# rchiaramo/wavefront_path_tracer

Measured on AMD Instinct MI355X. Metric: Mrays/s (extend+shade) at 1920×1080, 64 spp, 8 bounces; 1/2/4/8 GPU, higher is better.
Workload: dtype f32

## Files before the change

### wavefront_path_tracer_amd/_build.py

```python
import os
import shutil
import subprocess

PKG_DIR = os.path.dirname(os.path.abspath(__file__))
ROOT = os.path.dirname(PKG_DIR)
CSRC = os.path.join(PKG_DIR, "csrc")
LIB_PATH = os.path.join(PKG_DIR, "libwfpt.so")
SOURCES = ["wfpt_kernels.hip", "wfpt_api.hip", "wfpt_bvh_build.hip", "wfpt_host.cpp"]
HEADERS = [os.path.join(CSRC, "wfpt_kernels.h"), os.path.join(CSRC, "wfpt_bvh4.h"), os.path.join(CSRC, "wfpt_device_math.h"), os.path.join(CSRC, "wfpt_tile_lists.h"), os.path.join(CSRC, "wfpt_first_schedule.h"),
           os.path.join(ROOT, "include", "wfpt.h")]
FLAGS = ["--offload-arch=gfx950", "-O3", "-std=c++17", "-fPIC", "-shared", "-ffp-contract=off",
         "-fhip-fp32-correctly-rounded-divide-sqrt", "-fno-fast-math", "-Wall", "-Wno-unused-function"]


def hipcc():
    exe = shutil.which("hipcc") or "/opt/rocm/bin/hipcc"
    if not os.path.exists(exe):
        raise RuntimeError("hipcc not found: libwfpt.so cannot be built (and there is no CPU fallback)")
    return exe


def stale():
    if not os.path.exists(LIB_PATH):
        return True
    t = os.path.getmtime(LIB_PATH)
    deps = [os.path.join(CSRC, s) for s in SOURCES] + HEADERS + [os.path.abspath(__file__)]
    return any(os.path.getmtime(d) > t for d in deps)


BUILD_INFO = os.path.join(PKG_DIR, "build_info.json")


def source_digest():
    import hashlib
    h = hashlib.sha256()
    for f in [os.path.join(CSRC, s) for s in SOURCES] + HEADERS:
        h.update(os.path.basename(f).encode() + b"\0")
        h.update(open(f, "rb").read())
    return h.hexdigest()


def write_build_info():
    import datetime
    import json

    def git(*a):
        try:
            return subprocess.run(["git", "-C", ROOT] + list(a), stdout=subprocess.PIPE, stderr=subprocess.DEVNULL, text=True, timeout=20).stdout.strip()
        except Exception:
            return ""
    info = {"git_head": git("rev-parse", "HEAD") or None, "git_dirty": bool(git("status", "--porcelain", "--untracked-files=no")),
            "built_utc": datetime.datetime.utcnow().strftime("%Y-%m-%dT%H:%M:%SZ"), "source_sha256": source_digest(),
            "flags": FLAGS + os.environ.get("WFPT_EXTRA_FLAGS", "").split()}
    try:
        json.dump(info, open(BUILD_INFO, "w"), indent=1)
    except OSError:
        pass
    return info


def build_info():
    import json
    try:
        info = json.load(open(BUILD_INFO))
    except Exception:
        info = {"git_head": None}
    try:
        info["sources_match_build"] = info.get("source_sha256") == source_digest()
    except OSError:
        info["sources_match_build"] = None
    return info


def build(force=False, verbose=False):
    if not force and not stale():
        return LIB_PATH
    out = os.environ.get("WFPT_LIB_OUT", LIB_PATH)
    cmd = [hipcc()] + FLAGS + os.environ.get("WFPT_EXTRA_FLAGS", "").split()
    cmd += ["-I" + os.path.join(ROOT, "include"), "-I" + CSRC, "-o", out]
    cmd += [os.path.join(CSRC, s) for s in SOURCES]
    if verbose:
        print(" ".join(cmd))
    res = subprocess.run(cmd, stdout=subprocess.PIPE, stderr=subprocess.STDOUT, text=True)
    if res.returncode != 0:
        raise RuntimeError("hipcc failed:\n" + res.stdout)
    if verbose and res.stdout.strip():
        print(res.stdout)
    if out == LIB_PATH:
        write_build_info()
    return out


if __name__ == "__main__":
    print(build(force=True, verbose=True))
```

### wavefront_path_tracer_amd/csrc/wfpt_kernels.h

```cpp
#pragma once
#include <hip/hip_runtime.h>
#include <stddef.h>
#include <stdint.h>

#include "wfpt.h"
#include "wfpt_bvh4.h"
#include "wfpt_device_math.h"
#include "wfpt_first_schedule.h"
#include "wfpt_tile_lists.h"

namespace wfpt {

#ifndef WFPT_CHUNK
#define WFPT_CHUNK 512
#endif
constexpr int kChunk = WFPT_CHUNK;
constexpr int kExtendThreads = kChunk;
constexpr int kExtendWaves = kExtendThreads / 64;
#ifndef WFPT_CONSUMER_THREADS
#define WFPT_CONSUMER_THREADS 256
#endif
constexpr int kConsumerThreads = WFPT_CONSUMER_THREADS;
constexpr int kScanThreads = 1024;
constexpr int kMaxRows = 64;
constexpr int kMaxTrailDepth = 63;
constexpr int kMaxBatch = 128;
constexpr int kClsMax = 8;
constexpr int kMaxBatchClassic = 64;

struct Stride32 {
    uint32_t v;
    __host__ __device__ operator size_t() const { return v; }
    __host__ __device__ Stride32 &operator=(size_t x) { v = static_cast<uint32_t>(x); return *this; }
};

struct RayQueue {
    float *base;
    uint32_t cap;
    __host__ __device__ float *ox() const { return base; }
    __host__ __device__ float *oy() const { return base + cap; }
    __host__ __device__ float *oz() const { return base + 2u * static_cast<size_t>(cap); }
    __host__ __device__ float *dx() const { return base + 3u * static_cast<size_t>(cap); }
    __host__ __device__ float *dy() const { return base + 4u * static_cast<size_t>(cap); }
    __host__ __device__ float *dz() const { return base + 5u * static_cast<size_t>(cap); }
    __host__ __device__ uint32_t *pixel() const { return reinterpret_cast<uint32_t *>(base + 6u * static_cast<size_t>(cap)); }
};

struct HitQueue {
    uint32_t *base;
    Stride32 plane;
    __host__ __device__ float *t() const { return reinterpret_cast<float *>(base); }
    __host__ __device__ uint32_t *prim() const { return base + static_cast<size_t>(plane); }
    __host__ __device__ uint32_t *ridx() const { return base + 2u * static_cast<size_t>(plane); }
};
struct MissQueue {
    uint32_t *base;
    Stride32 plane;
    __host__ __device__ uint32_t *ridx() const { return base; }
    __host__ __device__ float *dy() const { return reinterpret_cast<float *>(base + static_cast<size_t>(plane)); }
    __host__ __device__ uint32_t *pixel() const { return base + 2u * static_cast<size_t>(plane); }
    __host__ __device__ float *dx() const { return reinterpret_cast<float *>(base + 3u * static_cast<size_t>(plane)); }
    __host__ __device__ float *dz() const { return reinterpret_cast<float *>(base + 4u * static_cast<size_t>(plane)); }
};
constexpr uint32_t kMissPlanes = 3, kMissPlanesEnv = 5;

struct EnvDev {
    const float4 *texels;
    uint32_t w, h;
    float intensity, rotation;
};

constexpr uint32_t kNoTexture = 0xffffffffu;
struct TexScene {
    const uint2 *prim_tex;
    const TexDev *tex;
    const float *uv6;
};

struct Control {
    uint32_t counters[16];
    wfpt_frame_buffer frame;
    uint32_t n_in;
    uint32_t seg_n;
    uint32_t hits;
    uint32_t misses;
    uint32_t shade_n;
    uint32_t miss_n;
    uint32_t shade_gx;
    uint32_t done;
    uint32_t ticket;
    uint32_t bounce;
    uint32_t samples;
    uint32_t _pad;
    uint32_t cls_n[kClsMax];
    uint32_t n_segs, next_segs, _pad2[2];
    uint32_t rows[kMaxRows][4];
    unsigned long long totals[4];
    unsigned long long wave_totals[kMaxRows][3];
};

struct ShadeRec {
    float v[3];
    float fuzz;
    float albedo[3];
    float refract_index;
    uint32_t mat_type;
    uint32_t cost_class;
    uint32_t _pad[2];
};

struct SceneDev {
    const wfpt_bvh_node *nodes;
    const float4 *prim_geom;
    const uint16_t *pair_parent;
    const uint32_t *pair_parent32;
    const wfpt_sphere *spheres;
    const wfpt_triangle *triangles;
    const wfpt_material *materials;
    const float4 *shade_rec;
    uint32_t n_nodes, n_spheres, n_materials;
    uint32_t prim_kind;
    uint32_t lds_scene;
    uint32_t lds_bytes;
    uint32_t depth;
    const float4 *nodes4;
    uint32_t tile_n;
    uint32_t *stack_spill;
    uint32_t spill_stride;
    const float4 *nodes_ch;
    float safe_c[3], safe_r2;
    uint32_t exact;
    uint32_t root_leaf;
};

constexpr uint32_t kStack4Lds = 8;
constexpr uint32_t kTileNodesMax = 341;

struct CameraDev {
    wfpt_gpu_camera cam;
    float inv_proj[16];
    float view[16];
};

struct Tiling {
    uint32_t rank, world;
};

struct Batch {
    uint32_t n;
    uint32_t ctl_stride;
    Stride32 ray_stride;
    Stride32 queue_stride;
    Stride32 chunk_stride;
    Stride32 image_stride;
};

struct GenerateArgs {
    Batch batch;
    RayQueue q;
    float *image;
    Control *ctl;
    const CameraDev *camera;
    uint32_t gx, gy;
    uint32_t true_size;
    uint32_t reset_image;
    uint32_t set_n_in;
    uint32_t capacity;
    Tiling tile;
};

struct ExtendArgs {
    Batch batch;
    RayQueue q;
    HitQueue hq;
    MissQueue mq;
    uint32_t *chunk_hits, *chunk_miss;
    float4 *rec_out;
    Control *ctl;
    const uint32_t *n_in;
    uint32_t limit;
    uint32_t has_inactive;
    uint32_t partition;
    uint16_t *mat_list;
    uint32_t *chunk_mat;
    size_t mat_list_mstride;
    size_t chunk_mat_mstride;
    SceneDev scene;
};

struct ScanArgs {
    Batch batch;
    const uint32_t *chunk_hits, *chunk_miss;
    uint32_t *chunk_hit_base, *chunk_miss_base;
    Control *ctl;
    const uint32_t *n_in;
    uint32_t limit;
    uint32_t *first_seg;
    uint32_t fused;
    uint32_t miss_floor;
    uint32_t bounce;
};

constexpr int kBounceFirst = 0;
constexpr int kBounceMiddle = 1;
constexpr int kBounceLast = 2;
#ifndef WFPT_MISS_SEGS
#define WFPT_MISS_SEGS 16
#endif
constexpr int kMissSegsPerItem = WFPT_MISS_SEGS;
#ifndef WFPT_MISS_EVERY
#define WFPT_MISS_EVERY 0
#endif
constexpr uint32_t kMissEvery = WFPT_MISS_EVERY;
#ifndef WFPT_FIRST_STATIC_SHARE_NUM
#define WFPT_FIRST_STATIC_SHARE_NUM 1
#endif
#ifndef WFPT_FIRST_STATIC_SHARE_DEN
#define WFPT_FIRST_STATIC_SHARE_DEN 2
#endif
constexpr uint32_t kFirstStaticNum = WFPT_FIRST_STATIC_SHARE_NUM, kFirstStaticDen = WFPT_FIRST_STATIC_SHARE_DEN;
static_assert(kFirstStaticDen > 0 && kFirstStaticNum <= kFirstStaticDen, "the static share of the first launch's items lies in [0, 1]");

struct BounceArgs {
    Batch batch;
    unsigned long long *stamps;
    const float4 *rec_in;
    float4 *rec_out;
    const uint32_t *in_hits, *in_hit_base, *in_miss;
    const uint32_t *in_first_seg;
    uint32_t *out_hits, *out_miss;
    MissQueue mq_in, mq_out;
    float *image;
    Control *ctl;
    const CameraDev *camera;
    uint32_t gx, gy;
    uint32_t capacity;
    uint32_t rng_mode;
    uint32_t image_width;
    Tiling tile;
    SceneDev scene;
    const uint32_t *plan;
    uint32_t plan_seg_off, plan_miss_off;
    const uint2 *cls_table;
    const uint32_t *first_seg_cls;
    uint32_t *out_cls;
    const uint4 *tile_lists;
};

struct TileListArgs {
    const float4 *nodes_ch;
    uint32_t n_nodes;
    const CameraDev *camera;
    uint32_t gx, gy;
    uint32_t width, height;
    Tiling tile;
    uint32_t *records;
};

template <int K> struct ClsPack {
    static constexpr int kFields = K + 2, kWords = (kFields + 2) / 3;
};
constexpr int kBinClasses = 4;
static_assert(kBinClasses <= kClsMax && kChunk <= 1023, "a packed field must hold a segment's count");

struct ScanBinnedArgs {
    Batch batch;
    const uint32_t *chunk_hits, *chunk_miss, *chunk_cls;
    uint2 *cls_table;
    uint32_t *first_seg_cls;
    Control *ctl;
    const uint32_t *n_in;
    uint32_t limit, miss_floor, bounce;
};

struct PlanArgs {
    Batch batch;
    const Control *ctl;
    uint32_t *plan;
    uint32_t plan_seg_off, plan_miss_off;
    uint32_t last;
};

constexpr uint32_t kDenseMiss = 0xffffffffu, kDenseInactive = 0xfffffffeu;
#ifndef WFPT_TICKET_BLOCK
#define WFPT_TICKET_BLOCK 64
#endif
constexpr uint32_t kTicketBlock = WFPT_TICKET_BLOCK;
#ifndef WFPT_REFILL_IDLE_PRESHADED
#define WFPT_REFILL_IDLE_PRESHADED 24
#endif
#ifndef WFPT_REFILL_IDLE_FIRST_PRE
#define WFPT_REFILL_IDLE_FIRST_PRE 16
#endif
constexpr uint32_t kRefillIdlePreshaded = WFPT_REFILL_IDLE_PRESHADED, kRefillIdleFirstPre = WFPT_REFILL_IDLE_FIRST_PRE;

struct RefillArgs {
    Batch batch;
    unsigned long long *stamps;
    const float4 *rec_in;
    float4 *dense_out;
    const uint32_t *in_hits, *in_hit_base, *in_first_seg;
    float *image;
    Control *ctl;
    const CameraDev *camera;
    uint32_t gx, gy, capacity, rng_mode, image_width;
    Tiling tile;
    SceneDev scene;
};

struct CompactArgs {
    Batch batch;
    const float4 *dense_in;
    float4 *rec_out;
    MissQueue mq_out;
    uint32_t *out_hits, *out_miss;
    const Control *ctl;
    uint32_t capacity;
};

struct ShadeArgs {
    Batch batch;
    RayQueue q, ext;
    HitQueue hq;
    const uint32_t *chunk_hits, *chunk_hit_base;
    const float4 *rec_in;
    float *image;
    Control *ctl;
    const uint32_t *n_hits;
    uint32_t limit;
    uint32_t gx;
    uint32_t rng_mode;
    uint32_t material;
    uint32_t split;
    const uint16_t *mat_list;
    const uint32_t *chunk_mat;
    size_t mat_list_mstride, chunk_mat_mstride;
    uint32_t count_out;
    uint32_t image_width;
    SceneDev scene;
    Tiling tile;
};

struct MissArgs {
    Batch batch;
    RayQueue q;
    MissQueue mq;
    const uint32_t *chunk_miss, *chunk_miss_base;
    float *image;
    const Control *ctl;
    const uint32_t *n_miss;
    uint32_t limit;
    uint32_t image_width;
    Tiling tile;
};

struct HitWalk {
    Batch batch;
    const float4 *rec_in;
    const uint32_t *in_hits, *in_hit_base;
    RayQueue q;
    HitQueue hq;
    const uint32_t *n_hits;
    uint32_t limit;
    uint32_t material;
    uint32_t capacity;
    float *image;
    const Control *ctl;
    uint32_t image_width;
    Tiling tile;
    const float4 *shade_rec;
};

struct TextureArgs {
    HitWalk w;
// ... 196 lines not shown
```

### wavefront_path_tracer_amd/csrc/wfpt_kernels.hip

```cpp
#include "wfpt_kernels.h"
#include "wfpt_device_math.h"

#include <type_traits>

namespace wfpt {

namespace {

constexpr float kPi = 3.1415927f;

__device__ __forceinline__ uint32_t lane_id() { return threadIdx.x & 63u; }
__device__ __forceinline__ uint32_t mbcnt(unsigned long long mask) {
    return __builtin_amdgcn_mbcnt_hi(static_cast<uint32_t>(mask >> 32),
                                     __builtin_amdgcn_mbcnt_lo(static_cast<uint32_t>(mask), 0u));
}
__device__ __forceinline__ uint32_t umin(uint32_t a, uint32_t b) { return a < b ? a : b; }
__device__ __forceinline__ uint32_t umax(uint32_t a, uint32_t b) { return a > b ? a : b; }
__device__ __forceinline__ uint32_t uniform(uint32_t v) { return __builtin_amdgcn_readfirstlane(v); }

#define WFPT_AS_LDS __attribute__((address_space(3)))
#define WFPT_AS_GLOBAL __attribute__((address_space(1)))
typedef float v4f_ __attribute__((ext_vector_type(4)));
__device__ __forceinline__ float4 load4_lds(const float4 *p) {
    const v4f_ v = *(const WFPT_AS_LDS v4f_ *)p;
// ... 1748 lines not shown
    if (shade_stamps) { asm volatile("s_waitcnt vmcnt(0)" ::: "memory"); shade_stamps[1] = stamp_now(); }
#endif
    shade_record<SCATTER, true, true>(s, ra, rb, __float_as_uint(rb.w), h, fb, ox, oy, oz, dx, dy, dz, pixel_idx);
}

typedef uint32_t v4u_ __attribute__((ext_vector_type(4)));
#define WFPT_AS_CONSTANT __attribute__((address_space(4)))
template <int PRIM>
__device__ __forceinline__ bool trace_tile_list(const uint4 *record, uint32_t w0, const float4 *prim_geom, float ox, float oy, float oz, float dx,
                                                float dy, float dz, float &t_out, uint32_t &prim_out) {
    const float a = (dx * dx + dy * dy) + dz * dz;
    float nearest = 1e30f;
    uint32_t best = 0xffffffffu, best_leaf = 0;
    const WFPT_AS_CONSTANT v4u_ *rec = (const WFPT_AS_CONSTANT v4u_ *)reinterpret_cast<uintptr_t>(record);
    uint32_t w = w0;
    for (uint32_t q = 0; q < kTileListCap / 4u && w != 0u; ++q) {
        const v4u_ four = rec[q];
        const uint32_t ws[4] = {four.x, four.y, four.z, four.w};
#pragma unroll
        for (int k = 0; k < 4; ++k) {
            w = ws[k];
            if (w == 0u) break;
            visit_leaf<PRIM>(prim_geom, w & 0xffffu, w >> 16, w, ox, oy, oz, dx, dy, dz, a, nearest, best, best_leaf);
        }
    }
    leaf_box_verdict<PRIM>(prim_geom, best_leaf & 0xffffu, best_leaf >> 16, false, ox, oy, oz, dx, dy, dz, nearest, best);
    t_out = nearest;
    prim_out = best;
    return nearest < 1e30f;
}

constexpr int kTileListThreads = 256;
__global__ __launch_bounds__(kTileListThreads) void tile_lists_kernel(TileListArgs a) {
    const uint32_t lane = lane_id();
    const uint32_t tile = uniform(blockIdx.x * (kTileListThreads / 64u) + (threadIdx.x >> 6));
    if (tile >= a.gx * a.gy) return;
    uint32_t *rec = a.records + static_cast<size_t>(tile) * kTileListCap;
    uint32_t x0, y0;
    tile_origin(tile, a.gx, a.tile.rank, a.tile.world, x0, y0);
    const CameraDev &cam = *a.camera;
    const TileBundle b = tile_bundle(cam.cam, cam.inv_proj, cam.view, x0, y0, a.width, a.height);
    bool list = b.ok != 0u && __float_as_uint(a.nodes_ch[1].w) == 0u;
    uint32_t count = 0;
    for (uint32_t base = 0; base < a.n_nodes && list; base += 64u) {
        const uint32_t i = base + lane;
        uint32_t w = 0u;
        if (i < a.n_nodes) {
            const float4 c = a.nodes_ch[2u * i], h = a.nodes_ch[2u * i + 1u];
            w = tile_leaf_word(i, __float_as_uint(c.w), __float_as_uint(h.w));
            if (w != 0u && w != kTileNoList && !tile_bundle_reaches(b, c.x, c.y, c.z, h.x, h.y, h.z)) w = 0u;
        }
        const unsigned long long mask = __ballot(w != 0u);
        const uint32_t slot = count + mbcnt(mask);
        if (__ballot(w == kTileNoList) != 0ull) list = false;
        if (w != 0u && slot < kTileListCap) rec[slot] = w;
        count += static_cast<uint32_t>(__popcll(mask));
        if (count > kTileListCap) list = false;
    }
    if (lane < kTileListCap) {
        if (!list) rec[lane] = lane == 0u ? kTileNoList : 0u;
        else if (lane >= count) rec[lane] = 0u;
    }
}

struct TicketMap {
    uint32_t n_hit, every, n_mixed;
    __device__ __forceinline__ TicketMap(uint32_t n_hit_items, uint32_t n_items, bool mix) : n_hit(n_hit_items) {
        const uint32_t n_miss = n_items - n_hit_items;
        every = kMissEvery ? kMissEvery : uniform(umin(umax(n_hit_items / umax(n_miss, 1u), 1u), 62u)) + 1u;
        n_mixed = mix ? umin(n_miss, n_hit_items / (every - 1u)) : 0u;
    }
    __device__ __forceinline__ uint32_t item_of(uint32_t t) const {
        if (t < n_mixed * every) {
            const uint32_t k = t / every, r = t - k * every;
            return r == every - 1u ? n_hit + k : k * (every - 1u) + r;
        }
        const uint32_t u = t - n_mixed * every, rest_h = n_hit - n_mixed * (every - 1u);
        return u < rest_h ? n_mixed * (every - 1u) + u : n_hit + n_mixed + (u - rest_h);
    }
};

struct BounceLds {
    uint32_t *cnt;
    uint32_t *next;
    uint32_t *total;
    uint16_t *items_h;
    uint16_t *items_m;
    uint32_t *stack;
};
constexpr uint32_t kBounceMiscWords = 4u * kExtendWaves + 2u + 2u + kMaxBatch;
static_assert(kBounceMiscWords % 4u == 0, "the stack column area stays 16-byte aligned");

#define WFPT_MISS_ITEM(SMP, FIRST_SEG, N_SEGS)                                                                                         \
    {                                                                                                                                  \
        const uint32_t smp = (SMP), first_seg = (FIRST_SEG), n_segs = (N_SEGS);                                                        \
        const size_t qo = smp * a.batch.queue_stride, co = smp * a.batch.chunk_stride;                                                 \
        float *image = a.image + smp * a.batch.image_stride;                                                                           \
        for (uint32_t k = wave; k < kMissSegsPerItem; k += kExtendWaves) {                                                             \
            const uint32_t seg = first_seg + k;                                                                                        \
            if (seg >= n_segs) break;                                                                                                  \
            const uint32_t count = uniform(a.in_miss[co + seg]);                                                                       \
            for (uint32_t r = lane; r < count; r += 64u) {                                                                             \
                const size_t slot = qo + static_cast<size_t>(seg) * kChunk + r;                                                        \
                const float dy = a.mq_in.dy()[slot];                           \
                const uint32_t pixel_idx = a.mq_in.pixel()[slot];                                                                      \
                const float3_ c = sky(dy);                                                                                             \
                float4 *px = pixel_of(image, local_pixel(pixel_idx, a.image_width, a.tile));                                           \
                const float4 thr = *px;                                                                                                \
                *px = make_float4(thr.x * c.x, thr.y * c.y, thr.z * c.z, thr.w);                                         \
            }                                                                                                                          \
        }                                                                                                                              \
    }

#ifndef WFPT_BOUNCE_ATTR
#define WFPT_BOUNCE_ATTR __launch_bounds__(kExtendThreads, WFPT_EXTEND_MIN_WAVES)
#endif
template <int MODE, typename Trail, int PRIM, bool LDS_SCENE, bool EXACT, bool ENV = false>
__global__ WFPT_BOUNCE_ATTR void bounce_kernel(BounceArgs a) {
    extern __shared__ float4 lds[];
    constexpr bool TRACE = MODE != kBounceLast;
    const bool stage_scene = TRACE && LDS_SCENE;
    WFPT_SCENE_LDS(stage_scene, s_misc);
    BounceLds L;
    L.cnt = s_misc;
    L.next = L.cnt + 4 * kExtendWaves;
    L.total = L.next + 2;
    L.items_h = reinterpret_cast<uint16_t *>(L.total + 2);
    L.items_m = L.items_h + kMaxBatch;
    L.stack = s_misc + kBounceMiscWords;

    const uint32_t n_slots = a.gx * a.gy * 64u;
    if (threadIdx.x < 2) L.total[threadIdx.x] = 0;
    __syncthreads();
    if (threadIdx.x < a.batch.n) {
        const uint32_t smp = threadIdx.x;
        const uint32_t n = MODE == kBounceFirst ? umin(n_slots, a.capacity) : umin(a.ctl[smp].shade_n, a.capacity);
        const uint32_t items_h = (n + kChunk - 1) / kChunk;
        uint32_t segs = 0;
        if (MODE != kBounceFirst && !ENV && a.ctl[smp].miss_n > 0) segs = (umin(a.ctl[smp].seg_n, a.capacity) + kChunk - 1) / kChunk;
        const uint32_t items_m = (segs + kMissSegsPerItem - 1) / kMissSegsPerItem;
        L.items_h[smp] = static_cast<uint16_t>(items_h);
        L.items_m[smp] = static_cast<uint16_t>(items_m);
        atomicAdd(&L.total[0], items_h);
        atomicAdd(&L.total[1], items_h + items_m);
    }
    __syncthreads();
    const uint32_t n_hit_items = uniform(L.total[0]), n_items = uniform(L.total[1]);
    uint32_t smp_h = 0, first_h = 0, smp_m = 0, first_m = n_hit_items;
    if (MODE == kBounceFirst && blockIdx.x == 0 && threadIdx.x < a.batch.n)
        a.ctl[threadIdx.x].n_in = umin(n_slots, a.capacity);
    const TicketMap tickets(n_hit_items, n_items, MODE != kBounceFirst);
    constexpr bool STATIC = MODE == kBounceFirst && kFirstStaticNum > 0;
    const uint32_t n_static = STATIC ? uniform(first_n_static(n_items, gridDim.x, kFirstStaticNum, kFirstStaticDen)) : 0u;
    uint32_t ticket = blockIdx.x;
    if (ticket >= n_items) return;
    uint32_t item = tickets.item_of(ticket);
    const float4 *g_nodes = reinterpret_cast<const float4 *>(a.scene.nodes);
    if (stage_scene) {
        WFPT_STAGE_SCENE(g_nodes);
        __syncthreads();
    }
    const wfpt_frame_buffer fb0 = uniform_frame(a.ctl);
    const uint32_t lane = lane_id(), wave = uniform(threadIdx.x >> 6);
    uint32_t iter = 0;
#if WFPT_STAMPS
    unsigned long long acc_cyc[4] = {0, 0, 0, 0}, acc_search = 0, acc_record = 0;
    unsigned long long acc_ticket = 0;
    uint32_t acc_cnt[5] = {0, 0, 0, 0, 0}, acc_drawn = 0;
#endif
    while (ticket < n_items) {
        const uint32_t buf = iter & 1u;
        const bool next_static = STATIC && first_next_is_static(ticket, n_static);
#if WFPT_STAMPS
        if (MODE == kBounceFirst && !next_static && wave == 0) {
            WFPT_STAMP(t_draw);
            uint32_t drawn = 0;
            if (threadIdx.x == 0) drawn = gridDim.x + atomicAdd(&a.ctl->ticket, 1u);
            asm volatile("s_waitcnt vmcnt(0)" ::: "memory");
            WFPT_STAMP(t_drawn);
            if (threadIdx.x == 0) L.next[buf] = drawn;
            acc_ticket += t_drawn - t_draw;
            acc_drawn += 1u;
        } else if (MODE != kBounceFirst)
#endif
        if (!next_static && threadIdx.x == 0) L.next[buf] = gridDim.x + atomicAdd(&a.ctl->ticket, 1u);
        if (!ENV && item >= n_hit_items) {
            while (item >= first_m + uniform(L.items_m[smp_m])) first_m += uniform(L.items_m[smp_m++]);
            WFPT_MISS_ITEM(smp_m, (item - first_m) * kMissSegsPerItem, (uniform(umin(a.ctl[smp_m].seg_n, a.capacity)) + kChunk - 1) / kChunk);
            __syncthreads();
            ticket = uniform(L.next[buf]);
            item = tickets.item_of(ticket);
            iter += 1;
            continue;
        }
        WFPT_STAMP(t_item);
        while (item >= first_h + uniform(L.items_h[smp_h])) first_h += uniform(L.items_h[smp_h++]);
        const uint32_t smp = smp_h;
        const uint32_t seg_out = item - first_h;
        const uint32_t n = MODE == kBounceFirst ? umin(n_slots, a.capacity) : uniform(umin(a.ctl[smp].shade_n, a.capacity));
        const size_t qo = smp * a.batch.queue_stride, co = smp * a.batch.chunk_stride;
        float *image = a.image + smp * a.batch.image_stride;
        wfpt_frame_buffer fb = fb0;
        fb.frame += smp;

        const uint32_t h = seg_out * kChunk + threadIdx.x;
        bool live = h < n;
        float ox = 0, oy = 0, oz = 0, dx = 0, dy = 0, dz = 0;
        uint32_t pixel_idx = 0;
        if (MODE == kBounceFirst) {
            const TilePixel p = tile_pixel(uniform(h >> 6), h, a.gx, a.tile);
            live = live && p.x < fb.width && p.y < fb.height;
            if (live) {
                WFPT_START_PATH(pr, p, fb, image, ox = pr.ox; oy = pr.oy; oz = pr.oz; dx = pr.dx; dy = pr.dy; dz = pr.dz);
            }
        } else if (live) {
            const HitSource src{a.rec_in, a.in_hit_base, a.in_first_seg, a.ctl + smp, image, a.scene.shade_rec, qo, co,
                                a.capacity, a.rng_mode, a.image_width, a.scene.prim_kind, a.tile};
#if WFPT_STAMPS
            unsigned long long sst[2] = {t_item, t_item};
            shade_hit<TRACE>(src, h, n, fb, ox, oy, oz, dx, dy, dz, pixel_idx, sst);
            if (MODE == kBounceMiddle) { acc_search += sst[0] - t_item; acc_record += sst[1] - sst[0]; }
#else
            shade_hit<TRACE>(src, h, n, fb, ox, oy, oz, dx, dy, dz, pixel_idx);
#endif
        }
        if (!TRACE) {
            __syncthreads();
            ticket = uniform(L.next[buf]);
            item = tickets.item_of(ticket);
            iter += 1;
            continue;
        }
        WFPT_STAMP(t_trace);
#if WFPT_STAMPS
        uint32_t dbg[3] = {0, 0, 0};
#endif
        float t = 0.0f;
        uint32_t prim = 0;
        bool hit = false;
        if (MODE == kBounceFirst && LDS_SCENE && !EXACT) {
            const uint4 *record = nullptr;
            uint32_t w0 = kTileNoList;
            if (a.tile_lists) {
                record = a.tile_lists + (kTileListCap / 4u) * uniform(h >> 6);
                w0 = uniform(*reinterpret_cast<const uint32_t *>(record));
            }
            if (w0 == kTileNoList) {
                if (live) WFPT_TRACE_ANY(g_nodes, L.stack, ox, oy, oz, dx, dy, dz);
            } else if (live) {
                prim = kHandOver;
                if (!far_origin(a.scene, ox, oy, oz)) hit = trace_tile_list<PRIM>(record, w0, s_geom, ox, oy, oz, dx, dy, dz, t, prim);
                if (prim == kHandOver)
                    hit = retrace_reference<Trail, PRIM, uint16_t>(g_nodes, s_geom, s_parent, ox, oy, oz, dx, dy, dz, a.scene.n_nodes, t, prim);
            }
        } else if (live) WFPT_TRACE_ANY(g_nodes, L.stack, ox, oy, oz, dx, dy, dz);
        WFPT_STAMP(t_traced);
        const bool miss = live && !hit;
        const unsigned long long hit_mask = __ballot(hit), miss_mask = __ballot(miss);
        if (lane == 0) {
            L.cnt[(buf * 2 + 0) * kExtendWaves + wave] = static_cast<uint32_t>(__popcll(hit_mask));
            L.cnt[(buf * 2 + 1) * kExtendWaves + wave] = static_cast<uint32_t>(__popcll(miss_mask));
        }
        __syncthreads();
        WFPT_STAMP(t_synced);
        uint32_t hit_before, miss_before, hit_total, miss_total;
        wave_offsets(L.cnt + buf * 2u * kExtendWaves, wave, lane, hit_before, hit_total, miss_before, miss_total);
        const size_t seg = qo + static_cast<size_t>(seg_out) * kChunk;
        if (hit) {
            float4 *rec = a.rec_out + 2u * (seg + hit_before);
            const uint32_t rank = mbcnt(hit_mask);
            rec[2u * rank] = make_float4(ox + t * dx, oy + t * dy, oz + t * dz, __uint_as_float(pixel_idx));
            rec[2u * rank + 1u] = make_float4(dx, dy, dz, __uint_as_float(prim));
        }
        if (miss) {
            const size_t first = seg + miss_before;
            const uint32_t rank = mbcnt(miss_mask);
            (a.mq_out.dy() + first)[rank] = dy;
            (a.mq_out.pixel() + first)[rank] = pixel_idx;
            if (ENV) {
                (a.mq_out.dx() + first)[rank] = dx;
                (a.mq_out.dz() + first)[rank] = dz;
            }
        }
        if (threadIdx.x == 0) {
            a.out_hits[co + seg_out] = hit_total;
            a.out_miss[co + seg_out] = miss_total;
        }
#if WFPT_STAMPS
        if (MODE == kBounceFirst) {
            WFPT_STAMP(t_done);
            acc_cyc[0] += t_trace - t_item;
            acc_cyc[1] += t_traced - t_trace;
            acc_cyc[2] += t_synced - t_traced;
            acc_cyc[3] += t_done - t_synced;
            acc_cnt[0] += 1u;
            acc_cnt[1] += static_cast<uint32_t>(__popcll(__ballot(live)));
        }
        if (MODE == kBounceMiddle) {
            asm volatile("s_waitcnt vmcnt(0)" ::: "memory");
            WFPT_STAMP(t_done);
            acc_cyc[0] += t_trace - t_item;
            acc_cyc[1] += t_traced - t_trace;
            acc_cyc[2] += t_synced - t_traced;
            acc_cyc[3] += t_done - t_synced;
            acc_cnt[0] += 1u;
            acc_cnt[1] += static_cast<uint32_t>(__popcll(__ballot(live)));
            uint32_t w_visits = dbg[0], w_leaves = dbg[1], l_visits = dbg[2];
            for (int d = 1; d < 64; d <<= 1) {
                w_visits = max(w_visits, static_cast<uint32_t>(__shfl_xor(w_visits, d, 64)));
                w_leaves = max(w_leaves, static_cast<uint32_t>(__shfl_xor(w_leaves, d, 64)));
                l_visits += static_cast<uint32_t>(__shfl_xor(l_visits, d, 64));
            }
            acc_cnt[2] += w_visits; acc_cnt[3] += w_leaves; acc_cnt[4] += l_visits;
        }
#endif
        if (next_static) ticket += gridDim.x;
        else ticket = first_dynamic_item(n_static, uniform(L.next[buf]));
        item = tickets.item_of(ticket);
        iter += 1;
    }
#if WFPT_STAMPS
    if (MODE == kBounceFirst && a.stamps && lane == 0) {
        for (int k = 0; k < 4; ++k) atomicAdd(&a.stamps[48 + k], acc_cyc[k]);
        atomicAdd(&a.stamps[48 + 4], static_cast<unsigned long long>(acc_cnt[0]));
        atomicAdd(&a.stamps[48 + 5], static_cast<unsigned long long>(acc_cnt[1]));
        if (wave == 0) {
            atomicAdd(&a.stamps[48 + 6], acc_ticket);
            atomicAdd(&a.stamps[48 + 7], static_cast<unsigned long long>(acc_drawn));
        }
    }
    if (MODE == kBounceMiddle && a.stamps && lane == 0) {
        for (int k = 0; k < 4; ++k) atomicAdd(&a.stamps[k], acc_cyc[k]);
        atomicAdd(&a.stamps[4], static_cast<unsigned long long>(acc_cnt[0]));
        atomicAdd(&a.stamps[5], static_cast<unsigned long long>(acc_cnt[1]));
        atomicAdd(&a.stamps[8], static_cast<unsigned long long>(acc_cnt[2]));
        atomicAdd(&a.stamps[9], static_cast<unsigned long long>(acc_cnt[3]));
        atomicAdd(&a.stamps[10], static_cast<unsigned long long>(acc_cnt[4]));
        atomicAdd(&a.stamps[11], acc_search);
        atomicAdd(&a.stamps[12], acc_record);
    }
#endif
}

template <int K> __device__ __forceinline__ uint32_t cls_field(const uint32_t *w, int f) { return (w[f / 3] >> (10 * (f % 3))) & 1023u; }

template <int MODE, typename Trail, int PRIM, bool EXACT, int K>
__global__ __launch_bounds__(kExtendThreads, WFPT_EXTEND_MIN_WAVES) void bounce_binned_kernel(BounceArgs a) {
    extern __shared__ float4 lds[];
    constexpr bool TRACE = MODE != kBounceLast;
    constexpr int NW = ClsPack<K>::kWords;
    constexpr bool LDS_SCENE = true;
    WFPT_SCENE_LDS(TRACE, s_cnt);
    uint32_t *s_next = s_cnt + 2 * kExtendWaves * NW;
    uint8_t *s_cls = reinterpret_cast<uint8_t *>(s_next + 2);

    const uint32_t nb = a.batch.n;
    const uint32_t n_slots = a.gx * a.gy * 64u;
    const uint32_t n_first = umin(n_slots, a.capacity), items_first = (n_first + kChunk - 1) / kChunk;
    const uint32_t *plan_h = a.plan, *plan_m = a.plan + a.plan_miss_off;
    if (MODE == kBounceLast) plan_h = a.plan + a.plan_seg_off;
    const uint32_t n_hit_items = MODE == kBounceFirst ? items_first * nb : uniform(plan_h[MODE == kBounceLast ? nb : nb * K]);
    const uint32_t n_items = MODE == kBounceFirst ? n_hit_items : uniform(plan_m[nb]);
    if (MODE == kBounceFirst && blockIdx.x == 0 && threadIdx.x < nb)
        a.ctl[threadIdx.x].n_in = n_first;
    const TicketMap tickets(n_hit_items, n_items, MODE != kBounceFirst);
    uint32_t ticket = blockIdx.x;
    if (ticket >= n_items) return;
    uint32_t item = tickets.item_of(ticket);
    const float4 *g_nodes = reinterpret_cast<const float4 *>(a.scene.nodes);
    if (TRACE) {
        WFPT_STAGE_SCENE(g_nodes);
        for (uint32_t i = threadIdx.x; i < a.scene.n_spheres; i += kExtendThreads)
            s_cls[i] = static_cast<uint8_t>(umin(__float_as_uint(a.scene.shade_rec[3u * i + 2u].y), static_cast<uint32_t>(K - 1)));
        __syncthreads();
    }
    const wfpt_frame_buffer fb0 = uniform_frame(a.ctl);
    const uint32_t lane = lane_id(), wave = uniform(threadIdx.x >> 6);
    uint32_t idx_h = 0, idx_m = 0;
    uint32_t iter = 0;
    while (ticket < n_items) {
        const uint32_t buf = iter & 1u;
        if (threadIdx.x == 0) s_next[buf] = gridDim.x + atomicAdd(&a.ctl->ticket, 1u);
        if (item >= n_hit_items) {
            while (item >= uniform(plan_m[idx_m + 1])) ++idx_m;
            WFPT_MISS_ITEM(idx_m, (item - uniform(plan_m[idx_m])) * kMissSegsPerItem, uniform(a.ctl[idx_m].n_segs));
            __syncthreads();
            ticket = uniform(s_next[buf]);
            item = tickets.item_of(ticket);
            iter += 1;
            continue;
        }
        uint32_t smp, seg_out;
        bool live;
        float ox = 0, oy = 0, oz = 0, dx = 0, dy = 0, dz = 0;
        uint32_t pixel_idx = 0;
        if (MODE == kBounceFirst) {
            smp = item / items_first;
            seg_out = item - smp * items_first;
        } else if (MODE == kBounceMiddle) {
            while (item >= uniform(plan_h[idx_h + 1])) ++idx_h;
            smp = idx_h / K;
            seg_out = item - uniform(plan_h[smp * K]);
        } else {
            while (item >= uniform(plan_h[idx_h + 1])) ++idx_h;
            smp = idx_h;
            seg_out = item - uniform(plan_h[idx_h]);
        }
        const size_t qo = smp * a.batch.queue_stride, co = smp * a.batch.chunk_stride;
        float *image = a.image + smp * a.batch.image_stride;
        wfpt_frame_buffer fb = fb0;
        fb.frame += smp;
        if (MODE == kBounceFirst) {
            const uint32_t h = seg_out * kChunk + threadIdx.x;
            const TilePixel p = tile_pixel(uniform(h >> 6), h, a.gx, a.tile);
            live = h < n_first && p.x < fb.width && p.y < fb.height;
            if (live) {
                WFPT_START_PATH(pr, p, fb, image, ox = pr.ox; oy = pr.oy; oz = pr.oz; dx = pr.dx; dy = pr.dy; dz = pr.dz);
            }
        } else {
            const HitSource src{a.rec_in, nullptr, nullptr, a.ctl + smp, image, a.scene.shade_rec, qo, co,
                                a.capacity, a.rng_mode, a.image_width, a.scene.prim_kind, a.tile};
            size_t slot = 0;
            if (MODE == kBounceMiddle) {
                const uint32_t k = idx_h - smp * K, run = item - uniform(plan_h[idx_h]);
                const uint32_t n_k = uniform(a.ctl[smp].cls_n[k]);
                const uint32_t q = run * kChunk + threadIdx.x;
                live = q < n_k;
                if (live) {
                    const uint32_t *fs = a.first_seg_cls + (static_cast<size_t>(smp) * K + k) * a.batch.chunk_stride;
                    uint32_t lo = uniform(fs[run]);
                    uint32_t hi = (run + 1u) * kChunk < n_k ? uniform(fs[run + 1u]) : uniform(a.ctl[smp].n_segs) - 1u;
                    const uint2 *tab = a.cls_table + co * K + k;
                    while (lo < hi) {
                        const uint32_t mid = (lo + hi + 1u) >> 1;
                        if (tab[static_cast<size_t>(mid) * K].x <= q) lo = mid; else hi = mid - 1u;
                    }
                    const uint2 e = tab[static_cast<size_t>(lo) * K];
                    slot = qo + e.y + (q - e.x);
                }
            } else {
                const uint32_t count = uniform(a.in_hits[co + seg_out]);
                live = threadIdx.x < count;
                slot = qo + static_cast<size_t>(seg_out) * kChunk + threadIdx.x;
            }
            if (live) {
                const float4 ra = a.rec_in[2u * slot], rb = a.rec_in[2u * slot + 1u];
                shade_record<TRACE, true, false>(src, ra, rb, __float_as_uint(rb.w), 0u, fb, ox, oy, oz, dx, dy, dz, pixel_idx);
            }
        }
        if (!TRACE) {
            __syncthreads();
            ticket = uniform(s_next[buf]);
            item = tickets.item_of(ticket);
            iter += 1;
            continue;
        }
#if WFPT_STAMPS
        uint32_t dbg[3] = {0, 0, 0};
#endif
        float t = 0.0f;
        uint32_t prim = 0;
        bool hit = false;
        if (live) WFPT_TRACE_ANY(g_nodes, static_cast<uint32_t *>(nullptr), ox, oy, oz, dx, dy, dz);
        const bool miss = live && !hit;
        const float hx = ox + t * dx, hy = oy + t * dy, hz = oz + t * dz;
        uint32_t cls = K;
        if (hit) cls = s_cls[prim];
        const unsigned long long hit_mask = __ballot(hit), miss_mask = __ballot(miss);
        uint32_t wcnt[NW];
#pragma unroll
        for (int j = 0; j < NW; ++j) wcnt[j] = 0;
        uint32_t rank = 0;
#pragma unroll
// ... 1683 lines not shown
```

Measured before the change: 25860.

## Draw dynamic tickets in chunks with single-item tail rounds, drop static first share

Each block's dynamic work-queue draw now claims a chunk of consecutive items (default four) instead of one. The last few grid-sized rounds stay single-item so load balance is kept at the end. The first-bounce static share default is set to zero so the first launch uses the same chunked dynamic scheme. This cuts per-item atomic/LDS ticket traffic and synchronisation overhead, but coarser grants risk more imbalance and worse locality of item order.

```diff
diff --git a/wavefront_path_tracer_amd/_build.py b/wavefront_path_tracer_amd/_build.py
--- a/wavefront_path_tracer_amd/_build.py
+++ b/wavefront_path_tracer_amd/_build.py
@@ -7,7 +7,7 @@
 CSRC = os.path.join(PKG_DIR, "csrc")
 LIB_PATH = os.path.join(PKG_DIR, "libwfpt.so")
 SOURCES = ["wfpt_kernels.hip", "wfpt_api.hip", "wfpt_bvh_build.hip", "wfpt_host.cpp"]
-HEADERS = [os.path.join(CSRC, "wfpt_kernels.h"), os.path.join(CSRC, "wfpt_bvh4.h"), os.path.join(CSRC, "wfpt_device_math.h"), os.path.join(CSRC, "wfpt_tile_lists.h"), os.path.join(CSRC, "wfpt_first_schedule.h"),
+HEADERS = [os.path.join(CSRC, "wfpt_kernels.h"), os.path.join(CSRC, "wfpt_bvh4.h"), os.path.join(CSRC, "wfpt_device_math.h"), os.path.join(CSRC, "wfpt_tile_lists.h"), os.path.join(CSRC, "wfpt_first_schedule.h"), os.path.join(CSRC, "wfpt_ticket_chunks.h"),
            os.path.join(ROOT, "include", "wfpt.h")]
 FLAGS = ["--offload-arch=gfx950", "-O3", "-std=c++17", "-fPIC", "-shared", "-ffp-contract=off",
          "-fhip-fp32-correctly-rounded-divide-sqrt", "-fno-fast-math", "-Wall", "-Wno-unused-function"]
diff --git a/wavefront_path_tracer_amd/csrc/wfpt_kernels.h b/wavefront_path_tracer_amd/csrc/wfpt_kernels.h
--- a/wavefront_path_tracer_amd/csrc/wfpt_kernels.h
+++ b/wavefront_path_tracer_amd/csrc/wfpt_kernels.h
@@ -7,6 +7,7 @@
 #include "wfpt_bvh4.h"
 #include "wfpt_device_math.h"
 #include "wfpt_first_schedule.h"
+#include "wfpt_ticket_chunks.h"
 #include "wfpt_tile_lists.h"
 
 namespace wfpt {
@@ -213,13 +214,28 @@
 #endif
 constexpr uint32_t kMissEvery = WFPT_MISS_EVERY;
 #ifndef WFPT_FIRST_STATIC_SHARE_NUM
-#define WFPT_FIRST_STATIC_SHARE_NUM 1
+#define WFPT_FIRST_STATIC_SHARE_NUM 0
 #endif
 #ifndef WFPT_FIRST_STATIC_SHARE_DEN
 #define WFPT_FIRST_STATIC_SHARE_DEN 2
 #endif
 constexpr uint32_t kFirstStaticNum = WFPT_FIRST_STATIC_SHARE_NUM, kFirstStaticDen = WFPT_FIRST_STATIC_SHARE_DEN;
 static_assert(kFirstStaticDen > 0 && kFirstStaticNum <= kFirstStaticDen, "the static share of the first launch's items lies in [0, 1]");
+#ifndef WFPT_FIRST_CHUNK
+#define WFPT_FIRST_CHUNK 4
+#endif
+#ifndef WFPT_FIRST_TAIL_ROUNDS
+#define WFPT_FIRST_TAIL_ROUNDS 4
+#endif
+#ifndef WFPT_BOUNCE_CHUNK
+#define WFPT_BOUNCE_CHUNK 4
+#endif
+#ifndef WFPT_BOUNCE_TAIL_ROUNDS
+#define WFPT_BOUNCE_TAIL_ROUNDS 4
+#endif
+constexpr uint32_t kFirstChunk = WFPT_FIRST_CHUNK, kFirstTailRounds = WFPT_FIRST_TAIL_ROUNDS;
+constexpr uint32_t kBounceChunk = WFPT_BOUNCE_CHUNK, kBounceTailRounds = WFPT_BOUNCE_TAIL_ROUNDS;
+static_assert(kFirstChunk >= 1 && kBounceChunk >= 1, "a draw buys at least one position");
 
 struct BounceArgs {
     Batch batch;
diff --git a/wavefront_path_tracer_amd/csrc/wfpt_kernels.hip b/wavefront_path_tracer_amd/csrc/wfpt_kernels.hip
--- a/wavefront_path_tracer_amd/csrc/wfpt_kernels.hip
+++ b/wavefront_path_tracer_amd/csrc/wfpt_kernels.hip
@@ -1924,7 +1924,12 @@
     const TicketMap tickets(n_hit_items, n_items, MODE != kBounceFirst);
     constexpr bool STATIC = MODE == kBounceFirst && kFirstStaticNum > 0;
     const uint32_t n_static = STATIC ? uniform(first_n_static(n_items, gridDim.x, kFirstStaticNum, kFirstStaticDen)) : 0u;
+    constexpr uint32_t CHUNK = MODE == kBounceFirst ? kFirstChunk : kBounceChunk, TAIL_ROUNDS = MODE == kBounceFirst ? kFirstTailRounds : kBounceTailRounds;
+    constexpr bool CHUNKED = CHUNK > 1;
+    const uint32_t n_dynamic = n_items - n_static;
+    const uint32_t chunk_end = CHUNKED ? uniform(chunk_body(n_dynamic, gridDim.x, CHUNK, TAIL_ROUNDS)) : 0u;
     uint32_t ticket = blockIdx.x;
+    if (CHUNKED && n_static == 0u) ticket = chunk_draw_position(ticket, n_dynamic, chunk_end, CHUNK);
     if (ticket >= n_items) return;
     uint32_t item = tickets.item_of(ticket);
     const float4 *g_nodes = reinterpret_cast<const float4 *>(a.scene.nodes);
@@ -1940,9 +1945,19 @@
     unsigned long long acc_ticket = 0;
     uint32_t acc_cnt[5] = {0, 0, 0, 0, 0}, acc_drawn = 0;
 #endif
+#define WFPT_NEXT_TICKET(DRAWN)                                                                                                        \
+    if (in_static) {                                                                                                                   \
+        ticket += gridDim.x;                                                                                                           \
+        if (CHUNKED && ticket >= n_static) ticket = n_static + chunk_draw_position(ticket - n_static, n_dynamic, chunk_end, CHUNK);    \
+    } else if (in_chunk) ticket += 1u;                                                                                                 \
+    else if (CHUNKED) ticket = n_static + chunk_draw_position(DRAWN, n_dynamic, chunk_end, CHUNK);                                     \
+    else ticket = first_dynamic_item(n_static, DRAWN);                                                                                 \
+    item = tickets.item_of(ticket);
     while (ticket < n_items) {
         const uint32_t buf = iter & 1u;
-        const bool next_static = STATIC && first_next_is_static(ticket, n_static);
+        const bool in_static = STATIC && first_next_is_static(ticket, n_static);
+        const bool in_chunk = CHUNKED && !in_static && chunk_follows(ticket - n_static, chunk_end, CHUNK);
+        const bool next_static = in_static || in_chunk;
 #if WFPT_STAMPS
         if (MODE == kBounceFirst && !next_static && wave == 0) {
             WFPT_STAMP(t_draw);
@@ -1960,8 +1975,12 @@
             while (item >= first_m + uniform(L.items_m[smp_m])) first_m += uniform(L.items_m[smp_m++]);
             WFPT_MISS_ITEM(smp_m, (item - first_m) * kMissSegsPerItem, (uniform(umin(a.ctl[smp_m].seg_n, a.capacity)) + kChunk - 1) / kChunk);
             __syncthreads();
-            ticket = uniform(L.next[buf]);
-            item = tickets.item_of(ticket);
+            if (MODE == kBounceFirst) {
+                ticket = uniform(L.next[buf]);
+                item = tickets.item_of(ticket);
+            } else {
+                WFPT_NEXT_TICKET(uniform(L.next[buf]));
+            }
             iter += 1;
             continue;
         }
@@ -1998,8 +2017,7 @@
         }
         if (!TRACE) {
             __syncthreads();
-            ticket = uniform(L.next[buf]);
-            item = tickets.item_of(ticket);
+            WFPT_NEXT_TICKET(uniform(L.next[buf]));
             iter += 1;
             continue;
         }
@@ -2086,11 +2104,10 @@
             acc_cnt[2] += w_visits; acc_cnt[3] += w_leaves; acc_cnt[4] += l_visits;
         }
 #endif
-        if (next_static) ticket += gridDim.x;
-        else ticket = first_dynamic_item(n_static, uniform(L.next[buf]));
-        item = tickets.item_of(ticket);
+        WFPT_NEXT_TICKET(uniform(L.next[buf]));
         iter += 1;
     }
+#undef WFPT_NEXT_TICKET
 #if WFPT_STAMPS
     if (MODE == kBounceFirst && a.stamps && lane == 0) {
         for (int k = 0; k < 4; ++k) atomicAdd(&a.stamps[48 + k], acc_cyc[k]);
diff --git a/wavefront_path_tracer_amd/csrc/wfpt_ticket_chunks.h b/wavefront_path_tracer_amd/csrc/wfpt_ticket_chunks.h
--- /dev/null
+++ b/wavefront_path_tracer_amd/csrc/wfpt_ticket_chunks.h
@@ -0,0 +1,26 @@
+#pragma once
+#include <stdint.h>
+
+#if defined(__HIP__)
+#define WFPT_TC_FN __host__ __device__ constexpr
+#else
+#define WFPT_TC_FN constexpr
+#endif
+
+namespace wfpt {
+
+WFPT_TC_FN uint32_t chunk_tail(uint32_t d, uint32_t grid, uint32_t tail_rounds) {
+    const uint64_t t = static_cast<uint64_t>(grid) * tail_rounds;
+    return t < d ? static_cast<uint32_t>(t) : d;
+}
+WFPT_TC_FN uint32_t chunk_body(uint32_t d, uint32_t grid, uint32_t chunk, uint32_t tail_rounds) {
+    return chunk * ((d - chunk_tail(d, grid, tail_rounds)) / chunk);
+}
+WFPT_TC_FN uint32_t chunk_draws(uint32_t d, uint32_t body, uint32_t chunk) { return body / chunk + (d - body); }
+WFPT_TC_FN uint32_t chunk_draw_position(uint32_t u, uint32_t d, uint32_t body, uint32_t chunk) {
+    const uint32_t n_body = body / chunk;
+    return u < n_body ? chunk * u : (u - n_body < d - body ? body + (u - n_body) : d);
+}
+WFPT_TC_FN bool chunk_follows(uint32_t p, uint32_t body, uint32_t chunk) { return p < body && p % chunk != chunk - 1u; }
+
+}
```

Result: faster. 27040, median of 6 (+4.6%).
